# pacargile/ThePayne

Measured on AMD Instinct MI355X. Metric: likelihood-evals/sec (4k-pixel ANN, 512 live points), higher is better.
Workload: dtype f32; 1 GPU; C2: single star per GPU, 4096-pixel 2x300 YST1 ANN, 3600 observed pixels, batch of 512 candidate vectors per step (dynesty live points); batch=512, npix=4096, nobs=3600, stars=1, kernel_variant=0, parallelism=1 star per GPU, no data-path collective, products=2 x fp16 parts, 3 products, fp32 accumulator

## Files before the change

thepayne_amd/csrc/dense_kernels.hpp:

```cpp
#pragma once

#include "sed_core.hpp"
#include "sampler_core.hpp"

typedef float f32x16 __attribute__((ext_vector_type(16)));
typedef float f32x4_t __attribute__((ext_vector_type(4)));

struct DenseParams {
  const float* X; int ldx;
  const float* W; int K;
  const float* Wd; int ldwd;
  int dma_tiles;
  int k_real;
  const float* bias;
  float* Y; int ldy;
  int B, N;
  float bias_shift;
  int act;
  int grid_m, grid_n;
  const double* theta; int ld_theta;
  const float* W0; const float* b0; int n_labels; int act0;
  int K0;
  unsigned short* Yp; const unsigned short* Xp; const unsigned short* Wp;
  int ldp; size_t plane_y, plane_x, plane_w;
  double xmin[PAYNE_MAX_LABELS], xden[PAYNE_MAX_LABELS];
  const unsigned long long* sel; unsigned long long sel_seq;
  const unsigned short* Wp_alt; size_t plane_w_alt; const float* bias_alt; float bias_shift_alt; int N_alt, ldy_alt;
  const float* W_alt;
  int yp_half; float yp_scale;
  const float* rscale; const float* rscale_alt;
  const unsigned short* Wh; size_t plane_wh; const float* rs1; float a0_scale; int h2_tiles;
#ifdef PAYNE_STAMPS
  unsigned long long* stamps;
#endif
};
#define PAYNE_HK_LEAD_PARAMS const void* lead_p0, const float* lead_p1, const float* lead_p2, const float* lead_bias, unsigned lead_i0, unsigned lead_i1, \
                             unsigned lead_i2, int lead_B, unsigned lead_i4, int lead_N
#define PAYNE_HK_LEAD_TYPES const void*, const float*, const float*, const float*, unsigned, unsigned, unsigned, int, unsigned, int
#define PAYNE_D3_LEAD_PARAMS const unsigned long long* lead_sel, const unsigned short* lead_Xp, const unsigned short* lead_Wp, unsigned lead_plane_x, \
                             unsigned lead_plane_w, unsigned lead_grid, int lead_N, int lead_B, int lead_ldp, int lead_K, unsigned lead_sel_seq
#define PAYNE_D3_LEAD_TYPES const unsigned long long*, const unsigned short*, const unsigned short*, unsigned, unsigned, unsigned, int, int, int, int, unsigned
#define PAYNE_D3_LEAD_ARGS(p) (p).sel, (p).Xp, (p).Wp, (unsigned)(p).plane_x, (unsigned)(p).plane_w, ((unsigned)(p).grid_m | ((unsigned)(p).grid_n << 16)), \
                              (p).N, (p).B, (p).ldp, (p).K, (unsigned)(p).sel_seq
#ifdef PAYNE_STAMPS
#ifdef PAYNE_STAMPS_ENDS_ONLY
#define HK_STAMP(k) do { if (((k) == 0 || (k) == 5 || (k) == 15) && p.stamps && threadIdx.x == 0) p.stamps[(size_t)blockIdx.x * 16 + (k)] = __builtin_amdgcn_s_memtime(); } while (0)
#else
#define HK_STAMP(k) do { if (p.stamps && threadIdx.x == 0) p.stamps[(size_t)blockIdx.x * 16 + (k)] = __builtin_amdgcn_s_memtime(); } while (0)
#endif
static unsigned long long* g_hidden_stamps = nullptr;
static unsigned long long* g_dense_stamps = nullptr;
#else
#define HK_STAMP(k) do {} while (0)
#endif

__device__ __forceinline__ float lrelu01(float z) { return fmaxf(z, 0.01f * z); }
__device__ __forceinline__ float sigmoid_f32(float z) {
  const float t = __builtin_amdgcn_fmed3f(-z, -88.0f, 88.0f);
  const float n = __builtin_rintf(t * 1.44269502f);
  float f = __builtin_fmaf(t, 1.44269502f, -n);
  f = __builtin_fmaf(t, 1.92596299e-8f, f);
  const float e = __builtin_amdgcn_ldexpf(__builtin_amdgcn_exp2f(f), (int)n);
  const float d = 1.0f + e;
  float r = __builtin_amdgcn_rcpf(d);
  r = __builtin_fmaf(__builtin_fmaf(-d, r, 1.0f), r, r);
  return z != z ? z : r;
}
__device__ __forceinline__ float act_apply(float z, int act) {
  if (act == PAYNE_ACT_SIGMOID) return sigmoid_f32(z);
  const float l = lrelu01(z);
  return act == PAYNE_ACT_LRELU ? l : z;
}

__device__ __forceinline__ void lds_barrier() { asm volatile("s_waitcnt lgkmcnt(0)\n\ts_barrier" ::: "memory"); }

template <int BM, int BN, int BK>
constexpr size_t dense_lds_bytes() { return (size_t)(2 * (BM + BN) * (BK + 4) + BM * PAYNE_MAX_LABELS) * sizeof(float); }

template <int BM, int BN, int BK, bool FUSE_L0>
__global__ void __launch_bounds__(256) payne_dense_kernel(DenseParams p) {
  constexpr int PITCH = BK + 4;
  constexpr int WM = BM / 2, WN = BN / 2;
  constexpr int TM = WM / 32, TN = WN / 32;
  constexpr int KQ = BK / 4;
  constexpr int A_F4 = BM * KQ / 256, B_F4 = BN * KQ / 256;
  extern __shared__ __attribute__((aligned(16))) float dk_sm[];
  float (*As)[BM * PITCH] = reinterpret_cast<float (*)[BM * PITCH]>(dk_sm);
  float (*Bs)[BN * PITCH] = reinterpret_cast<float (*)[BN * PITCH]>(dk_sm + 2 * BM * PITCH);
  float* Xh = dk_sm + 2 * (BM + BN) * PITCH;

  const int ntiles = p.grid_m * p.grid_n;
  int t = blockIdx.x;
  if ((ntiles & 7) == 0) t = (t & 7) * (ntiles >> 3) + (t >> 3);
  const int m0 = (t % p.grid_m) * BM, n0 = (t / p.grid_m) * BN;
  const int tid = threadIdx.x, lane = tid & 63, wave = tid >> 6;
  const int wm0 = (wave >> 1) * WM, wn0 = (wave & 1) * WN;

  if (FUSE_L0) {
    for (int idx = tid; idx < BM * p.n_labels; idx += 256) {
      const int r = idx / p.n_labels, d = idx - r * p.n_labels, row = m0 + r;
      float v = 0.f;
      if (row < p.B) {
        const double x = p.theta[(size_t)row * p.ld_theta + (d < 4 ? d : 6)];
        v = (float)((x - p.xmin[d]) / p.xden[d] - 0.5);
      }
      Xh[r * PAYNE_MAX_LABELS + d] = v;
// ... 476 lines not shown
#endif
    frags((it + 1) % NS, fn);
    __builtin_amdgcn_sched_barrier(0);
    if (it + AHEAD < nk) issue((it + AHEAD) % NS, (it + AHEAD) * KD);
    __builtin_amdgcn_sched_barrier(0);
  };
  auto epilogue = [&]() {
  if (col < p.N) {
    const bool act_none = __builtin_amdgcn_readfirstlane(p.act == PAYNE_ACT_NONE ? 1 : 0) != 0;
    if (act_none && m0 + 64 <= p.B) {
      const unsigned voff = 4u * ((unsigned)(4 * (lane >> 5)) * (unsigned)p.ldy + (unsigned)col);
      const unsigned char* yb = reinterpret_cast<const unsigned char*>(p.Y + (size_t)(m0 + wm0) * p.ldy);
#pragma unroll
      for (int r = 0; r < 16; ++r) {
        const unsigned char* rowp = yb + (size_t)((r & 3) + 8 * (r >> 2)) * p.ldy * 4;
        d2_store_row(reinterpret_cast<float*>(const_cast<unsigned char*>(rowp + voff)), __builtin_fmaf(acc[r], rs, bv));
      }
    } else if (act_none) {
#pragma unroll
      for (int r = 0; r < 16; ++r) {
        const int row = m0 + wm0 + (r & 3) + 8 * (r >> 2) + 4 * (lane >> 5);
        if (row < p.B) d2_store_row(&p.Y[(size_t)row * p.ldy + col], __builtin_fmaf(acc[r], rs, bv));
      }
    } else {
#pragma unroll
      for (int r = 0; r < 16; ++r) {
        const int row = m0 + wm0 + (r & 3) + 8 * (r >> 2) + 4 * (lane >> 5);
        if (row < p.B) __builtin_nontemporal_store(act_apply(__builtin_fmaf(acc[r], rs, bv), p.act), &p.Y[(size_t)row * p.ldy + col]);
      }
    }
  }
  };
  int it = 0;
#pragma unroll
  for (; it + 2 < nk; it += 2) {
    head(it, f1, f0);
    all_products(f0);
    __builtin_amdgcn_sched_barrier(0);
    head(it + 1, f0, f1);
    all_products(f1);
    __builtin_amdgcn_sched_barrier(0);
  }
  if (it + 1 < nk) {
    head(it, f1, f0);
    all_products(f0);
    last_products(f1);
  } else {
    last_products(f0);
  }
  epilogue();
  HK_STAMP(15);
}

template <int NK> constexpr size_t d2hh_lds_bytes() { return (size_t)NK * 16384 + 3 * 16384; }
template <int NK>
__global__ void __launch_bounds__(512) payne_dense_dma2hh_kernel(PAYNE_D3_LEAD_PARAMS, DenseParams p_) {
  DenseParams p = p_;
  p.sel = lead_sel; p.Xp = lead_Xp; p.Wp = lead_Wp; p.plane_x = lead_plane_x; p.plane_w = lead_plane_w;
  p.grid_m = (int)(lead_grid & 0xffffu); p.grid_n = (int)(lead_grid >> 16); p.N = lead_N; p.B = lead_B; p.ldp = lead_ldp; p.K = lead_K;
  constexpr int KD = 64, ROWB = 2 * KD, CPR = ROWB / 16, RPP = 1024 / ROWB;
  constexpr int PLANE = 64 * ROWB, STAGE = 2 * PLANE;
  constexpr int NSB = 3, AHEAD = 2, KS = KD / 16, NT = 2 * NK;
  constexpr int RING = NK * STAGE;
  auto sw = [](int row) { return (row >> 1) & 7; };
  extern __shared__ __attribute__((aligned(16))) unsigned char d2_sm[];
  if (p.sel != nullptr && (unsigned)*p.sel == lead_sel_seq) {
    p.Wp = p.Wp_alt; p.plane_w = p.plane_w_alt; p.bias = p.bias_alt; p.bias_shift = p.bias_shift_alt; p.N = p.N_alt; p.ldy = p.ldy_alt;
    p.rscale = p.rscale_alt;
  }
  const int ntiles = p.grid_m * p.grid_n;
  int t = blockIdx.x;
  if ((ntiles & 7) == 0) t = (t & 7) * (ntiles >> 3) + (t >> 3);
  const int m0 = (t % p.grid_m) * 64, n0 = (t / p.grid_m) * 128;
  if (n0 >= p.N) return;
  const int tid = threadIdx.x, lane = tid & 63;
  const int wave = __builtin_amdgcn_readfirstlane(tid >> 6);
  const int half = wave >> 2, w4 = wave & 3;
  const int wm0 = (w4 >> 1) * 32, wn0 = 64 * half + (w4 & 1) * 32;
  const int lrow = lane / CPR, lchunk = lane % CPR;
  const unsigned pitch_a = 2u * (unsigned)p.ldp, pitch_b = 2u * (unsigned)p.K;
  const unsigned char* sb1[4]; unsigned vo1[4]; int ds1[4];
  const unsigned char* sb2[4]; unsigned vo2[4]; int ds2[4];
#pragma unroll
  for (int j = 0; j < 4; ++j) {
    {
      const bool isA = j < 2;
      const int pl = j & 1, blk = wave;
      const int row = RPP * blk + lrow, c = lchunk ^ sw(row);
      const int top = isA ? p.B - 1 - m0 : p.N - 1 - n0;
      const int r = (isA ? m0 : n0) + (row < top ? row : top);
      sb1[j] = isA ? reinterpret_cast<const unsigned char*>(p.Xp) + 2 * (size_t)pl * p.plane_x
                   : reinterpret_cast<const unsigned char*>(p.Wp) + 2 * (size_t)pl * p.plane_w;
      vo1[j] = (unsigned)r * (isA ? pitch_a : pitch_b) + 16u * (unsigned)c;
      ds1[j] = pl * PLANE + blk * 1024;
    }
    {
      const int pl = j >> 1, blk = 2 * w4 + (j & 1);
      const int row = RPP * blk + lrow, c = lchunk ^ sw(row);
      const int top = p.N - 1 - n0;
      const int r = n0 + (64 + row < top ? 64 + row : top);
      sb2[j] = reinterpret_cast<const unsigned char*>(p.Wp) + 2 * (size_t)pl * p.plane_w;
      vo2[j] = (unsigned)r * pitch_b + 16u * (unsigned)c;
      ds2[j] = pl * PLANE + blk * 1024;
    }
  }
  auto issue = [&](int q) {
    if (q < NK) {
#pragma unroll
      for (int j = 0; j < 4; ++j)
        __builtin_amdgcn_global_load_lds((const __attribute__((address_space(1))) void*)(sb1[j] + vo1[j] + 2 * KD * q),
                                         (__attribute__((address_space(3))) void*)(d2_sm + (j < 2 ? q * STAGE : RING + (q % NSB) * STAGE) + ds1[j]), 16, 0, 0);
    } else if (half) {
#pragma unroll
      for (int j = 0; j < 4; ++j)
        __builtin_amdgcn_global_load_lds((const __attribute__((address_space(1))) void*)(sb2[j] + vo2[j] + 2 * KD * (q - NK)),
                                         (__attribute__((address_space(3))) void*)(d2_sm + RING + (q % NSB) * STAGE + ds2[j]), 16, 0, 0);
    }
  };
  f32x16 acc;
#pragma unroll
  for (int r = 0; r < 16; ++r) acc[r] = 0.f;
  const int Ra = wm0 + (lane & 31), Rb = (w4 & 1) * 32 + (lane & 31), h = lane >> 5;
  const int sa = sw(Ra), sb = sw(Rb);
  struct Frag { f16x8_t a[KS][2], b[KS][2]; };
  auto frags = [&](int q, Frag& f) {
    const unsigned char* As = d2_sm + (q < NK ? q : q - NK) * STAGE;
    const unsigned char* Bs = d2_sm + RING + (q % NSB) * STAGE;
#pragma unroll
    for (int ks = 0; ks < KS; ++ks) {
      const int c = 2 * ks + h;
#pragma unroll
      for (int pl = 0; pl < 2; ++pl) {
        f.a[ks][pl] = *reinterpret_cast<const f16x8_t*>(As + pl * PLANE + Ra * ROWB + 16 * (c ^ sa));
        f.b[ks][pl] = *reinterpret_cast<const f16x8_t*>(Bs + pl * PLANE + Rb * ROWB + 16 * (c ^ sb));
      }
    }
  };
  auto products = [&](const Frag& f, int ks) {
    acc = __builtin_amdgcn_mfma_f32_32x32x16_f16(f.a[ks][1], f.b[ks][0], acc, 0, 0, 0);
    acc = __builtin_amdgcn_mfma_f32_32x32x16_f16(f.a[ks][0], f.b[ks][1], acc, 0, 0, 0);
    acc = __builtin_amdgcn_mfma_f32_32x32x16_f16(f.a[ks][0], f.b[ks][0], acc, 0, 0, 0);
  };
  const int k_tail = (p.k_real > 0 ? p.k_real : p.K) - (NK - 1) * KD;
  const int ks_last = __builtin_amdgcn_readfirstlane((k_tail + 15) >> 4);
  auto stage_products = [&](const Frag& f, bool last) {
#pragma unroll
    for (int ks = 0; ks < KS; ++ks)
      if (!last || ks < ks_last) products(f, ks);
  };
  const int col = n0 + wn0 + (lane & 31);
  const float bv = p.bias[col < p.N ? col : p.N - 1] - p.bias_shift;
  const float rs = p.rscale[col < p.N ? col : p.N - 1];
  auto epilogue = [&]() {
    if (col >= p.N) return;
    const bool act_none = __builtin_amdgcn_readfirstlane(p.act == PAYNE_ACT_NONE ? 1 : 0) != 0;
    if (act_none && m0 + 64 <= p.B) {
      const unsigned voff = 4u * ((unsigned)(4 * (lane >> 5)) * (unsigned)p.ldy + (unsigned)col);
      const unsigned char* yb = reinterpret_cast<const unsigned char*>(p.Y + (size_t)(m0 + wm0) * p.ldy);
#pragma unroll
      for (int r = 0; r < 16; ++r) {
        const unsigned char* rowp = yb + (size_t)((r & 3) + 8 * (r >> 2)) * p.ldy * 4;
        d2_store_row(reinterpret_cast<float*>(const_cast<unsigned char*>(rowp + voff)), __builtin_fmaf(acc[r], rs, bv));
      }
    } else {
#pragma unroll
      for (int r = 0; r < 16; ++r) {
        const int row = m0 + wm0 + (r & 3) + 8 * (r >> 2) + 4 * (lane >> 5);
        if (row < p.B) {
          const float y = __builtin_fmaf(acc[r], rs, bv);
          __builtin_nontemporal_store(act_none ? y : act_apply(y, p.act), &p.Y[(size_t)row * p.ldy + col]);
        }
      }
    }
  };
  HK_STAMP(0);
  Frag f0, f1;
  if (half == 0) {
    issue(0); issue(1);
    asm volatile("s_waitcnt vmcnt(4)" ::: "memory");
    asm volatile("s_barrier" ::: "memory");
    frags(0, f0);
#pragma unroll
    for (int q = 0; q + 1 < NK; ++q) {
      Frag& fc = (q & 1) ? f1 : f0;
      Frag& fn = (q & 1) ? f0 : f1;
      asm volatile("s_waitcnt vmcnt(0)" ::: "memory");
      asm volatile("s_barrier" ::: "memory");
      HK_STAMP(1 + q);
      frags(q + 1, fn);
      __builtin_amdgcn_sched_barrier(0);
      if (q + AHEAD < NK) issue(q + AHEAD);
      __builtin_amdgcn_sched_barrier(0);
      stage_products(fc, false);
      __builtin_amdgcn_sched_barrier(0);
    }
    asm volatile("s_barrier" ::: "memory");
    stage_products(((NK - 1) & 1) ? f1 : f0, true);
    HK_STAMP(NK);
    epilogue();
    HK_STAMP(15);
    return;
  }
  issue(0); issue(1);
  asm volatile("s_waitcnt vmcnt(4)" ::: "memory");
  asm volatile("s_barrier" ::: "memory");
#pragma unroll
  for (int q = 0; q + 1 < NK; ++q) {
    asm volatile("s_waitcnt vmcnt(0)" ::: "memory");
    asm volatile("s_barrier" ::: "memory");
    issue(q + AHEAD);
  }
  asm volatile("s_waitcnt vmcnt(0)" ::: "memory");
  asm volatile("s_barrier" ::: "memory");
  frags(NK, f0);
  __builtin_amdgcn_sched_barrier(0);
  if (NK + 1 < NT) issue(NK + 1);
  __builtin_amdgcn_sched_barrier(0);
#pragma unroll
  for (int q = NK; q < NT; ++q) {
    Frag& fc = ((q - NK) & 1) ? f1 : f0;
    Frag& fn = ((q - NK) & 1) ? f0 : f1;
    if (q + 1 < NT) {
      asm volatile("s_waitcnt vmcnt(0)" ::: "memory");
      asm volatile("s_barrier" ::: "memory");
      frags(q + 1, fn);
      __builtin_amdgcn_sched_barrier(0);
      if (q + AHEAD < NT) issue(q + AHEAD);
      __builtin_amdgcn_sched_barrier(0);
    }
    stage_products(fc, q == NT - 1);
    __builtin_amdgcn_sched_barrier(0);
  }
  epilogue();
  HK_STAMP(15);
}

constexpr int D3_STAGE = 3 * (64 + 128) * 64;
template <int NS> constexpr size_t d3_lds_bytes() { return (size_t)NS * D3_STAGE; }
template <int NK, int NS, bool PIPE>
__global__ void __launch_bounds__(512) payne_dense_dma3_kernel(PAYNE_D3_LEAD_PARAMS, DenseParams p_) {
  DenseParams p = p_;
  p.sel = lead_sel; p.Xp = lead_Xp; p.Wp = lead_Wp; p.plane_x = lead_plane_x; p.plane_w = lead_plane_w;
  p.grid_m = (int)(lead_grid & 0xffffu); p.grid_n = (int)(lead_grid >> 16); p.N = lead_N; p.B = lead_B; p.ldp = lead_ldp; p.K = lead_K;
  constexpr int D3_NS = NS, AHEAD = PIPE ? D3_NS - 1 : 1;
  static_assert((PIPE && NS >= 3) || (!PIPE && NS == 2 && NK == 0), "ring depth / schedule");
  extern __shared__ __attribute__((aligned(16))) unsigned char d3_sm[];
  if (p.sel != nullptr && (unsigned)*p.sel == lead_sel_seq) {
    p.Wp = p.Wp_alt; p.plane_w = p.plane_w_alt; p.bias = p.bias_alt; p.bias_shift = p.bias_shift_alt; p.N = p.N_alt; p.ldy = p.ldy_alt;
  }
  const int ntiles = p.grid_m * p.grid_n;
  int t = blockIdx.x;
  if ((ntiles & 7) == 0) t = (t & 7) * (ntiles >> 3) + (t >> 3);
  const int m0 = (t % p.grid_m) * 64, n0 = (t / p.grid_m) * 128;
  if (n0 >= p.N) return;
  const int tid = threadIdx.x, lane = tid & 63;
  const int wave = __builtin_amdgcn_readfirstlane(tid >> 6);
  const int wm0 = (wave >> 2) * 32, wn0 = (wave & 3) * 32;
  const bool five = wave < 4;
  const unsigned char* src[5];
  int dst[5];
#pragma unroll
  for (int j = 0; j < 5; ++j) {
    int q = five ? wave * 5 + j : 20 + (wave - 4) * 4 + j;
    if (q > 35) q = 35;
    const bool isA = q < 12;
    const int pl = isA ? q >> 2 : (q - 12) >> 3, blk = isA ? (q & 3) : ((q - 12) & 7);
    const int row = 16 * blk + (lane >> 2);
    const int c = (lane & 3) ^ ((row >> 2) & 3);
    if (isA) {
      const int r = (m0 + row < p.B) ? m0 + row : p.B - 1;
      src[j] = reinterpret_cast<const unsigned char*>(p.Xp + (size_t)pl * p.plane_x + (size_t)r * p.ldp) + 16 * c;
      dst[j] = pl * 4096 + blk * 1024;
    } else {
      const int r = (n0 + row < p.N) ? n0 + row : p.N - 1;
      src[j] = reinterpret_cast<const unsigned char*>(p.Wp + (size_t)pl * p.plane_w + (size_t)r * p.K) + 16 * c;
      dst[j] = 3 * 4096 + pl * 8192 + blk * 1024;
    }
  }
  auto issue = [&](int stage, int k0) {
#pragma unroll
    for (int j = 0; j < 5; ++j)
      if (j < 4 || five)
        __builtin_amdgcn_global_load_lds((const __attribute__((address_space(1))) void*)(src[j] + 2 * k0),
                                         (__attribute__((address_space(3))) void*)(d3_sm + stage * D3_STAGE + dst[j]), 16, 0, 0);
  };
  auto wait_landed = [&](int younger) {
    if (younger <= 0) asm volatile("s_waitcnt vmcnt(0)" ::: "memory");
// ... 1229 lines not shown
```

thepayne_amd/csrc/payne_hip.hip:

```cpp
#include <hip/hip_runtime.h>

#include <chrono>
#include <cstdio>
#include <cstdlib>
#include <cstring>
#include <string>
#include <thread>
#include <vector>

#include "../../include/payne_hip.h"
#include "host_tables.hpp"
#include "post_seq.hpp"
#include "ns_core.hpp"

using namespace payne;

#include "dense_kernels.hpp"

#include "post_kernels.hpp"

#include "sed_kernel.hpp"
#include "select.hpp"

__global__ void payne_photonly_kernel(const double* mags, const double* obs, const double* err, int F, int B, double* lnl) {
  const int b = blockIdx.x * blockDim.x + threadIdx.x;
  if (b < B) lnl[b] = -0.5 * sed_chi2(mags + (size_t)b * F, obs, err, F);
}

static std::string g_create_error;

struct payne_ctx {
  int device = 0;
  payne_opts opts{};
  std::string err;
  std::vector<void*> owned;
  std::vector<void*> obs_owned;
  bool has_model = false;
  int n_layers = 0;
  payne_layer layers[PAYNE_MAX_LAYERS];
  int n_labels = 0;
  double xmin[PAYNE_MAX_LABELS], xden[PAYNE_MAX_LABELS];
  HostTables H;
  PostTables T{};
  float* hid[2] = {nullptr, nullptr};
  int ld_hid = 0;
  float* raw = nullptr;
  const float* w_out_pad = nullptr;
  const float* w_hid_pad[PAYNE_MAX_LAYERS] = {};
  int w_out_kp = 0;
  bool dma_ok = false;
  unsigned short* w_out_p3 = nullptr; unsigned short* hid_p3 = nullptr;
  unsigned short* w_out_p3z = nullptr; const float* bias_z = nullptr; bool freq_ok = false;
  const float* w_out_padz = nullptr;
  unsigned short* w_out_h2 = nullptr; unsigned short* w_out_h2z = nullptr; const float* rscale = nullptr; const float* rscalez = nullptr;
  float act_scale = 0.f;
  unsigned short* w1_h2 = nullptr; const float* rs1 = nullptr; float a0_scale = 0.f; int w1_rows = 0;
  unsigned short* wl_h2[PAYNE_MAX_LAYERS] = {}; const float* rsl[PAYNE_MAX_LAYERS] = {}; float hs[PAYNE_MAX_LAYERS] = {};
  unsigned short* hid_h2[2] = {nullptr, nullptr};
  unsigned long long* chain_flags = nullptr; unsigned long long chain_calls = 0;
  bool freq_rs = false; unsigned long long* rot_flag = nullptr; unsigned long long rot_seq = 0;
  size_t post_lds = 0;
  void (*post_fn_lean)(PAYNE_POST_SIG) = nullptr;
  bool post_tw_lds = false;
  int n_cu = 256;
  bool lean_available = false;
  PostTables* d_T = nullptr;
  post_kernel_fn post_fn = nullptr;
  float* big_ws = nullptr;
  int big_grid = 0;
  bool big_tiled = false;
  bool big_chip = false;
  bool big_chip2 = false;
  bool has_cont = false;
  int cn_layers = 0, cn_npix = 0, cn_ld_hid = 0;
  payne_layer clayers[PAYNE_MAX_LAYERS];
  double cxmin[PAYNE_MAX_LABELS], cxden[PAYNE_MAX_LABELS];
  float* chid[2] = {nullptr, nullptr};
  float* cont_raw = nullptr;
  const double* cont_scale = nullptr;
  const int* cont_idx = nullptr;
  const double* cont_frac = nullptr;
  std::vector<void*> cont_owned;
  bool has_lsf = false;
  const double* d_obs_wave = nullptr;
  const double* lsf = nullptr;
  const double* lsf_wave = nullptr;
  int n_lsf = 0;
  float* lsf_spec = nullptr;
  double* lsf_ws = nullptr;
  float* lsf_fws = nullptr;
  bool lsf_global = false;
  int lsf_chunk = 0;
  std::vector<void*> lsf_owned;
  bool obs_bound = false;
  CandState* prep = nullptr;
  bool has_phot = false, has_obs_phot = false;
  PhotTables P{};
  double* mags_ws = nullptr;
  double *obs_mag = nullptr, *obs_err = nullptr;
  int ncols = 0;
  bool prof = false;
  struct ProfRec { hipEvent_t e0, e1; int kind; };
  std::vector<ProfRec> prof_pool;
// ... 132 lines not shown
  c->T.obs_min = c->H.obs_min;
  c->T.obs_max = c->H.obs_max;
  c->T.ln_obs_min = std::log(c->H.obs_min); c->T.ln_obs_max = std::log(c->H.obs_max);
  c->T.obs_sorted = 1;
  for (int i = 1; i < obs->nobs; ++i) if (!(obs->wave[i] >= obs->wave[i - 1])) { c->T.obs_sorted = 0; break; }
  c->obs_bound = true;
  return sync_tables(c);
}

extern "C" int payne_version(void) { return PAYNE_ABI_VERSION; }

extern "C" const char* payne_last_error(const payne_ctx* ctx) { return ctx ? ctx->err.c_str() : g_create_error.c_str(); }

extern "C" int payne_theta_cols(const payne_ctx* ctx) { return ctx ? ctx->ncols : PAYNE_E_INVALID; }

extern "C" const char* payne_kernel_name(int which) {
  switch (which) {
    case 0: return "payne_dense_kernel";
    case 1: return "payne_post_kernel";
    case 2: return "payne_sed_kernel";
    default: return "";
  }
}

__global__ void payne_activation_kernel(const float* __restrict__ z, int n, int act, float* __restrict__ out) {
  const int i = blockIdx.x * blockDim.x + threadIdx.x;
  if (i < n) out[i] = act_apply(z[i], act);
}
extern "C" int payne_activation_batch(const float* z, int n, int act, float* out, void* stream) {
  if (!z || !out || n < 0 || act < PAYNE_ACT_NONE || act > PAYNE_ACT_SIGMOID) return PAYNE_E_INVALID;
  if (n == 0) return PAYNE_OK;
  hipLaunchKernelGGL(payne_activation_kernel, dim3((n + 255) / 256), dim3(256), 0, reinterpret_cast<hipStream_t>(stream), z, n, act, out);
  return hipGetLastError() == hipSuccess ? PAYNE_OK : PAYNE_E_HIP;
}
extern "C" const char* payne_last_kernel(const payne_ctx* c, int kind) {
  if (c && kind == 4) return c->last_rows_freq ? "frequency" : "pixels";
  return (c && kind >= 0 && kind < 4) ? c->last_kernel[kind] : "";
}

extern "C" void payne_ctx_destroy(payne_ctx* c) {
  if (!c) return;
  int prev = 0;
  (void)hipGetDevice(&prev);
  (void)hipSetDevice(c->device);
  for (void* p : c->owned) (void)hipFree(p);
  for (void* p : c->obs_owned) (void)hipFree(p);
  for (void* p : c->cont_owned) (void)hipFree(p);
  for (void* p : c->lsf_owned) (void)hipFree(p);
  for (auto& r : c->prof_pool) { (void)hipEventDestroy(r.e0); (void)hipEventDestroy(r.e1); }
  (void)hipSetDevice(prev);
  delete c;
}

static hipError_t set_dense_attributes();
static double hidden_amax(const payne_model_desc* m, std::string& why, double* per_layer = nullptr) {
  const int nl = m->n_layers, D = m->n_labels;
  if (nl < 3) { why = "no hidden layer pair"; return 0.0; }
  std::vector<std::vector<float>> W(nl - 1), b(nl - 1);
  for (int l = 0; l + 1 < nl; ++l) {
    const payne_layer& L = m->layers[l];
    W[l].resize((size_t)L.n_out * L.n_in); b[l].resize((size_t)L.n_out);
    if (hipMemcpy(W[l].data(), L.w, W[l].size() * 4, hipMemcpyDeviceToHost) != hipSuccess ||
        hipMemcpy(b[l].data(), L.b, b[l].size() * 4, hipMemcpyDeviceToHost) != hipSuccess) { why = "hipMemcpy"; return 0.0; }
  }
  auto act = [](double z, int a) { return a == PAYNE_ACT_LRELU ? (z > 0 ? z : 0.01 * z) : (a == PAYNE_ACT_SIGMOID ? 1.0 / (1.0 + std::exp(-z)) : z); };
  std::vector<std::vector<double>> pts;
  for (int cidx = 0; cidx < (1 << D); ++cidx) { std::vector<double> x(D); for (int d = 0; d < D; ++d) x[d] = ((cidx >> d) & 1) ? 0.6 : -0.6; pts.push_back(x); }
  pts.push_back(std::vector<double>(D, 0.0));
  unsigned long long st = 0x9E3779B97F4A7C15ull;
  for (int i = 0; i < 64; ++i) {
    std::vector<double> x(D);
    for (int d = 0; d < D; ++d) { st = st * 6364136223846793005ull + 1442695040888963407ull; x[d] = ((double)(st >> 11) / 9007199254740992.0 - 0.5) * 1.2; }
    pts.push_back(x);
  }
  double amax = 0.0;
  std::vector<double> a, y;
  for (const auto& x : pts) {
    a = x;
    for (int l = 0; l + 1 < nl; ++l) {
      const payne_layer& L = m->layers[l];
      y.assign((size_t)L.n_out, 0.0);
      for (int o = 0; o < L.n_out; ++o) {
        double z = b[l][o];
        const float* w = &W[l][(size_t)o * L.n_in];
        for (int k = 0; k < L.n_in; ++k) z += (double)w[k] * a[k];
        y[o] = act(z, L.act);
      }
      a.swap(y);
      if (per_layer) for (double v : a) { if (std::isfinite(v)) per_layer[l] = std::max(per_layer[l], std::fabs(v)); else per_layer[l] = 1e300; }
    }
    for (double v : a) { if (!std::isfinite(v)) { why = "non-finite activation"; return 0.0; } amax = std::max(amax, std::fabs(v)); }
  }
  return amax;
}
static int make_h2_planes(payne_ctx* c, const float* d_w, const std::vector<float>& h_w, int n, int kp, float act_scale,
                          unsigned short** planes, const float** rscale) {
  std::vector<float> sc((size_t)n), rs((size_t)n);
  for (int i = 0; i < n; ++i) {
    float mx = 0.f;
    for (int k = 0; k < kp; ++k) mx = std::max(mx, std::fabs(h_w[(size_t)i * kp + k]));
    int e = 0;
    if (mx > 0.f && std::isfinite(mx)) e = (int)std::floor(std::log2(16384.0 / (double)mx));
    e = std::max(-100, std::min(100, e));
    sc[i] = (float)std::ldexp(1.0, e);
    rs[i] = (float)(std::ldexp(1.0, -e) / (double)act_scale);
  }
  const float* d_sc = nullptr;
// ... 147 lines not shown
  if (!phot->w1 || !phot->b1 || !phot->w2 || !phot->b2 || !phot->w3 || !phot->b3 || !phot->xmin || !phot->xmax)
    return fail(c, PAYNE_E_INVALID, "phot descriptor has NULL members");
  PhotTables& P = c->P;
  const int F = phot->n_filters, H = phot->hidden;
  P.F = F; P.H = H;
  P.w1 = phot->w1; P.b1 = phot->b1; P.b2 = phot->b2; P.w3 = phot->w3; P.b3 = phot->b3;
  for (int d = 0; d < 6; ++d) { P.xmin[d] = phot->xmin[d]; P.xden[d] = phot->xmax[d] - phot->xmin[d]; }
  {
    std::vector<float> w2((size_t)F * H * H), w2t((size_t)F * H * H);
    he = hipMemcpy(w2.data(), phot->w2, w2.size() * 4, hipMemcpyDeviceToHost);
    if (he != hipSuccess) return fail(c, PAYNE_E_HIP, std::string("hipMemcpy(w2): ") + hipGetErrorString(he));
    for (int f = 0; f < F; ++f)
      for (int h = 0; h < H; ++h)
        for (int k = 0; k < H; ++k) w2t[((size_t)f * H + k) * H + h] = w2[((size_t)f * H + h) * H + k];
    if ((rc = upload(c, w2t, &P.w2t, c->owned))) return rc;
  }
  if (phot->hiav) {
    std::vector<double> hv(phot->hiav, phot->hiav + (size_t)F * 5);
    if ((rc = upload(c, hv, &P.hiav, c->owned))) return rc;
  }
  if (phot->obs_mag && phot->obs_err) {
    std::vector<double> m(phot->obs_mag, phot->obs_mag + F), e(phot->obs_err, phot->obs_err + F);
    const double *dm, *de;
    if ((rc = upload(c, m, &dm, c->owned))) return rc;
    if ((rc = upload(c, e, &de, c->owned))) return rc;
    c->obs_mag = const_cast<double*>(dm); c->obs_err = const_cast<double*>(de);
    c->has_obs_phot = true;
  }
  if ((rc = dev_alloc(c, (size_t)opts->b_max * F, &c->mags_ws, c->owned))) return rc;
  if ((size_t)H * 16 > 48 * 1024) {
    he = hipFuncSetAttribute(reinterpret_cast<const void*>(payne_sed_kernel), hipFuncAttributeMaxDynamicSharedMemorySize, H * 16);
    if (he != hipSuccess) return fail(c, PAYNE_E_HIP, std::string("hipFuncSetAttribute(sed): ") + hipGetErrorString(he));
  }
  c->has_phot = true;
  return PAYNE_OK;
}

extern "C" int payne_ctx_create(const payne_model_desc* model, const payne_obs_desc* obs, const payne_phot_desc* phot,
                                const payne_opts* opts, int device, payne_ctx** out) {
  if (!out) return fail(nullptr, PAYNE_E_INVALID, "out is NULL");
  *out = nullptr;
  if (!opts || opts->b_max <= 0) return fail(nullptr, PAYNE_E_INVALID, "opts.b_max must be > 0");
  if (opts->npoly < 0 || opts->npoly > PAYNE_MAX_POLY) return fail(nullptr, PAYNE_E_INVALID, "opts.npoly out of range");
  if (!model && !phot) return fail(nullptr, PAYNE_E_INVALID, "need a spectral model and/or a photometric model");
  hipError_t he = hipSetDevice(device);
  if (he != hipSuccess) return fail(nullptr, PAYNE_E_HIP, std::string("hipSetDevice: ") + hipGetErrorString(he));
  payne_ctx* c = new payne_ctx();
  c->device = device;
  { int ncu = 0; if (hipDeviceGetAttribute(&ncu, hipDeviceAttributeMultiprocessorCount, device) == hipSuccess && ncu > 0) c->n_cu = ncu; }
  c->opts = *opts;
  c->ncols = 8 + opts->npoly + 4;
  int rc = PAYNE_OK;
  auto bail = [&](int code) { g_create_error = c->err; payne_ctx_destroy(c); return code; };
  he = set_dense_attributes();
  if (he != hipSuccess) return bail(fail(c, PAYNE_E_HIP, std::string("hipFuncSetAttribute(dense): ") + hipGetErrorString(he)));

  if (model) {
    if (model->n_layers < 2 || model->n_layers > PAYNE_MAX_LAYERS) return bail(fail(c, PAYNE_E_INVALID, "model.n_layers must be 2..8"));
    if (model->n_labels < 1 || model->n_labels > PAYNE_MAX_LABELS) return bail(fail(c, PAYNE_E_INVALID, "model.n_labels must be 1..5"));
    if (!model->xmin || !model->xmax || !model->wavelength) return bail(fail(c, PAYNE_E_INVALID, "model.xmin/xmax/wavelength missing"));
    if (model->layers[0].n_in != model->n_labels) return bail(fail(c, PAYNE_E_INVALID, "first layer n_in != n_labels"));
    if (model->layers[model->n_layers - 1].n_out != model->npix) return bail(fail(c, PAYNE_E_INVALID, "last layer n_out != npix"));
    int maxh = 0;
    if ((rc = adopt_layers(c, model, c->layers, c->owned, "", &maxh))) return bail(rc);
    if ((rc = create_dense_operands(c, model, opts, maxh))) return bail(rc);
    c->n_layers = model->n_layers;
    c->n_labels = model->n_labels;
    for (int d = 0; d < model->n_labels; ++d) { c->xmin[d] = model->xmin[d]; c->xden[d] = model->xmax[d] - model->xmin[d]; }
    rc = build_model_tables(model->wavelength, model->npix, c->H);
    if (rc == -1) return bail(fail(c, PAYNE_E_INVALID, "model.npix must be >= 16"));
    if (rc == -2) return bail(fail(c, PAYNE_E_INVALID, "model.wavelength must be strictly increasing"));
    if (c->H.n1 > (1 << 20)) return bail(fail(c, PAYNE_E_UNSUPPORTED, "npix > 2^20"));
    PostTables& T = c->T;
    fill_model_scalars(c->H, T);
    T.r_ann = model->resolution; T.npoly = opts->npoly;
    if ((rc = upload(c, c->H.vs_tab32, &T.vs_tab, c->owned))) return bail(rc);
    T.vs_tab += 1;
    if ((rc = dev_alloc(c, 1, &c->d_T, c->owned))) return bail(rc);
    if ((rc = upload(c, c->H.lnlam, &T.lnlam, c->owned))) return bail(rc);
    if ((rc = upload(c, c->H.lam, &T.lam, c->owned))) return bail(rc);
    if ((rc = upload(c, c->H.tw, &T.tw, c->owned))) return bail(rc);
    if ((rc = upload(c, c->H.twf, &T.twf, c->owned))) return bail(rc);
    if ((rc = upload(c, c->H.rs1_idx, &T.rs1_idx, c->owned))) return bail(rc);
    if ((rc = upload(c, c->H.rs1_frac, &T.rs1_frac, c->owned))) return bail(rc);
    if ((rc = upload(c, c->H.bk1_idx, &T.bk1_idx, c->owned))) return bail(rc);
    if ((rc = upload(c, c->H.bk1_frac, &T.bk1_frac, c->owned))) return bail(rc);
    c->ld_hid = (maxh + 31) & ~31;
    if (model->n_layers > 2) {
      if ((rc = dev_alloc(c, (size_t)opts->b_max * c->ld_hid, &c->hid[0], c->owned))) return bail(rc);
      if ((rc = dev_alloc(c, (size_t)opts->b_max * c->ld_hid, &c->hid[1], c->owned))) return bail(rc);
      if (c->w_out_p3 && (rc = dev_alloc(c, (size_t)3 * opts->b_max * c->ld_hid, &c->hid_p3, c->owned))) return bail(rc);
    }
    if ((rc = dev_alloc(c, (size_t)opts->b_max * std::max(model->npix, T.n1 <= 16384 ? T.n1 : 0), &c->raw, c->owned, false))) return bail(rc);
    if ((rc = dev_alloc(c, (size_t)opts->b_max, &c->prep, c->owned, false))) return bail(rc);
    if (T.n1 > 16384) {
      c->big_grid = opts->b_max < 256 ? opts->b_max : 256;
      c->big_chip2 = T.n1 == kChip2N1 && c->H.geo && !(opts->variant & PAYNE_V_BIG_WORKSPACE);
      if ((rc = dev_alloc(c, (size_t)c->big_grid * (c->big_chip2 ? 4 : 2) * T.n1, &c->big_ws, c->owned, false))) return bail(rc);
      if (c->big_chip2) {
        he = hipFuncSetAttribute(reinterpret_cast<const void*>(payne_post_chip2_kernel), hipFuncAttributeMaxDynamicSharedMemorySize,
                                 (int)kChipLdsBytes);
        if (he != hipSuccess) return bail(fail(c, PAYNE_E_HIP, std::string("hipFuncSetAttribute(chip2): ") + hipGetErrorString(he)));
      }
      c->big_tiled = true;
      c->big_chip = T.n1 == kChipN1 && c->H.geo && !(opts->variant & PAYNE_V_BIG_WORKSPACE);
      if (c->big_chip) {
        he = hipFuncSetAttribute(reinterpret_cast<const void*>(payne_post_chip_kernel), hipFuncAttributeMaxDynamicSharedMemorySize,
// ... 78 lines not shown
  }
  if ((rc = upload(c, scale, &c->cont_scale, c->cont_owned))) return rc;
  if ((rc = upload(c, idx, &c->cont_idx, c->cont_owned))) return rc;
  if ((rc = upload(c, frac, &c->cont_frac, c->cont_owned))) return rc;
  c->has_cont = true;
  return PAYNE_OK;
}

static int set_lsf_impl(payne_ctx* c, const double* lsf_wave, const double* lsf, int n) {
  if (!c) return PAYNE_E_INVALID;
  if (!c->has_model) return fail(c, PAYNE_E_INVALID, "context has no spectral model");
  DeviceScope ds(c);
  for (void* p : c->lsf_owned) (void)hipFree(p);
  c->lsf_owned.clear();
  c->has_lsf = false;
  if (!lsf) return PAYNE_OK;
  if (!c->obs_bound) return fail(c, PAYNE_E_INVALID, "bind the observed grid before its LSF vector");
  if (!lsf_wave && n != c->T.nobs) return fail(c, PAYNE_E_INVALID, "the LSF vector must have one entry per observed pixel");
  if (lsf_wave && n < 2) return fail(c, PAYNE_E_INVALID, "an LSF vector on its own wavelengths needs at least two entries");
  for (int i = 0; i < n; ++i)
    if (!(lsf[i] > 0.0)) return fail(c, PAYNE_E_INVALID, "LSF dispersions must be positive");
  if (lsf_wave)
    for (int i = 1; i < n; ++i)
      if (!(lsf_wave[i] > lsf_wave[i - 1])) return fail(c, PAYNE_E_INVALID, "the LSF vector's wavelengths must be strictly increasing");
  std::vector<double> v(lsf, lsf + n);
  int rc;
  if ((rc = upload(c, v, &c->lsf, c->lsf_owned))) return rc;
  c->n_lsf = n;
  c->lsf_wave = c->d_obs_wave;
  if (lsf_wave) {
    std::vector<double> w(lsf_wave, lsf_wave + n);
    if ((rc = upload(c, w, &c->lsf_wave, c->lsf_owned))) return rc;
  }
  c->lsf_global = c->T.n1 > 8192 || (c->opts.variant & PAYNE_V_LSF_GLOBAL);
  c->lsf_chunk = c->lsf_global ? std::min(c->opts.b_max, 256) : c->opts.b_max;
  if ((rc = dev_alloc(c, (size_t)c->lsf_chunk * c->T.npix, &c->lsf_spec, c->lsf_owned, false))) return rc;
  if ((rc = dev_alloc(c, (size_t)c->lsf_chunk * (2 * (size_t)c->T.npix + c->T.n1), &c->lsf_ws, c->lsf_owned, false))) return rc;
  if (c->lsf_global) {
    if ((rc = dev_alloc(c, (size_t)c->lsf_chunk * 2 * fft_buf_floats(c->T.n1), &c->lsf_fws, c->lsf_owned, false))) return rc;
  } else {
    const size_t lds = (size_t)c->T.n1 * 8 + 2 * (size_t)fft_buf_floats(c->T.n1) * 4 + (256 + 8) * 8;
    hipError_t he = hipFuncSetAttribute(reinterpret_cast<const void*>(payne_lsf_kernel<false>), hipFuncAttributeMaxDynamicSharedMemorySize, (int)lds);
    if (he != hipSuccess) return fail(c, PAYNE_E_HIP, std::string("hipFuncSetAttribute: ") + hipGetErrorString(he));
  }
  c->has_lsf = true;
  return PAYNE_OK;
}
extern "C" int payne_ctx_set_lsf(payne_ctx* c, const double* lsf, int n) { return set_lsf_impl(c, nullptr, lsf, n); }
extern "C" int payne_ctx_set_lsf_on(payne_ctx* c, const double* lsf_wave, const double* lsf, int n) {
  if (c && lsf && !lsf_wave) return fail(c, PAYNE_E_INVALID, "lsf_wave is NULL");
  return set_lsf_impl(c, lsf_wave, lsf, n);
}

static hipError_t set_dense_attributes() {
  hipError_t e = hipSuccess;
  auto set = [&](const void* f, size_t lds) {
    const hipError_t r = hipFuncSetAttribute(f, hipFuncAttributeMaxDynamicSharedMemorySize, (int)lds);
    if (e == hipSuccess) e = r;
  };
#define PAYNE_SET_T(K, ARGS, ...) set(reinterpret_cast<const void*>(PAYNE_UNPAREN K), __VA_ARGS__);
#define PAYNE_SET_F(K, ...) set(reinterpret_cast<const void*>(K), __VA_ARGS__);
  PAYNE_DENSE_KERNELS(PAYNE_SET_T, PAYNE_SET_F)
  return e;
}

template <int BM, int BN, int BK, bool FUSE>
static void launch_dense(DenseParams& p, hipStream_t s) {
  p.grid_m = (p.B + BM - 1) / BM;
  p.grid_n = (p.N + BN - 1) / BN;
#ifdef PAYNE_STAMPS
  p.stamps = FUSE ? nullptr : g_dense_stamps;
#endif
  PAYNE_LAUNCH_DENSE((payne_dense_kernel<BM, BN, BK, FUSE>), dim3(p.grid_m * p.grid_n), dim3(256), s, p);
}

template <int BK, int NK, int NS, bool PIPE>
static void launch_out_dma_nk(DenseParams& p, hipStream_t s) {
  constexpr int WN = 4;
  PAYNE_LAUNCH_DENSE((payne_dense_dma_kernel<WN, BK, NK, NS, PIPE>), dim3(p.grid_m * p.grid_n), dim3(128 * WN), s, p);
}
struct OutPlan {
  OutForm form = OutForm::Generic;
  int grid_m = 0, grid_n = 0;
  bool sel = false;
  bool big = false;
  bool own_cu = false;
  bool fixed = false;
  bool bk64 = false;
  bool halves = false;
  bool split_w = false;
};
static void launch_out_dma(payne_ctx* c, DenseParams& p, hipStream_t s, const OutPlan& plan) {
  p.k_real = p.K;
  p.W = c->w_out_pad; p.K = c->w_out_kp;
  p.grid_m = plan.grid_m; p.grid_n = plan.grid_n;
#ifdef PAYNE_STAMPS
  p.stamps = g_dense_stamps;
#endif
  if (plan.bk64) {
    if (plan.fixed) launch_out_dma_nk<64, 5, 3, true>(p, s); else launch_out_dma_nk<64, 0, 3, true>(p, s);
  } else if (plan.own_cu) {
    if (plan.fixed) launch_out_dma_nk<32, 10, 4, true>(p, s); else launch_out_dma_nk<32, 0, 4, true>(p, s);
  } else {
    launch_out_dma_nk<32, 0, 3, false>(p, s);
  }
}

static void launch_out_planes(payne_ctx* c, DenseParams& p, hipStream_t s, const OutPlan& plan, bool freq) {
  const bool h2 = plan.form == OutForm::H2;
  p.k_real = p.K;
// ... 69 lines not shown
    else PAYNE_LAUNCH_DENSE((payne_dense_hidden_kernel<true, PAYNE_MAX_LABELS>), grid, block, s, PAYNE_HK_ARGS);
  }
#undef PAYNE_HK_ARGS
}

struct NetRef {
  const payne_layer* layers; int n_layers; int n_labels; const double* xmin; const double* xden;
  float* const* hid; int ld_hid; float* out; int ld_out; float out_shift;
  bool spectral;
  bool freq = false;
  bool sel = false;
};
static NetRef spectral_net(const payne_ctx* c) {
  return NetRef{c->layers, c->n_layers, c->n_labels, c->xmin, c->xden, c->hid, c->ld_hid, c->raw, c->T.npix, kBase, true};
}
static NetRef continuum_net(const payne_ctx* c) {
  return NetRef{c->clayers, c->cn_layers, c->n_labels, c->cxmin, c->cxden, c->chid, c->cn_ld_hid, c->cont_raw, c->cn_npix, 0.f, false};
}
struct BatchRows {
  const float* rows = nullptr; int ld = 0;
  bool freq = false;
  bool sel = false; unsigned long long rot_seq = 0;
  const CandState* prep = nullptr;
  bool spec = false;
};
struct SpecReq { const WalkTail* walk; const WalkState* w; int step, K; };
static OutForm out_form(const payne_ctx* c, const NetRef& N) {
  OutForm f = wanted_out_form(c->opts.variant);
  if (!(N.spectral && c->dma_ok && c->ld_hid >= c->w_out_kp)) return OutForm::Generic;
  if (f >= OutForm::Bf16x3 && !(c->w_out_p3 && c->hid_p3)) f = OutForm::F32Dma;
  if (f == OutForm::H2) {
    const unsigned long long plane_w = 2ull * (unsigned long long)std::max(N.layers[N.n_layers - 1].n_out, c->T.n1) * (unsigned long long)c->w_out_kp;
    const unsigned long long plane_x = 2ull * (unsigned long long)c->opts.b_max * (unsigned long long)c->ld_hid;
    if (plane_w >= (1ull << 31) || plane_x >= (1ull << 31) || !c->w_out_h2 || !(c->act_scale > 0.f)) f = OutForm::Bf16x3;
  }
  return f;
}
static OutPlan plan_out(const payne_ctx* c, const NetRef& N, int B) {
  const unsigned v = c->opts.variant;
  const int kp = c->w_out_kp, n_out = N.layers[N.n_layers - 1].n_out;
  OutPlan o; o.sel = N.sel;
  const int n_launch = o.sel ? c->T.n1 : n_out;
  o.form = out_form(c, N);
  if (o.form == OutForm::H2 && N.freq && !c->w_out_h2z) o.form = OutForm::Bf16x3;
  if (o.form == OutForm::Generic) return o;
  o.grid_m = (B + 63) / 64; o.grid_n = (n_launch + 127) / 128;
  o.own_cu = o.grid_m * o.grid_n <= c->n_cu;
  o.fixed = kp == 320 && !(v & PAYNE_V_OUT_ROLLED);
  if (o.form == OutForm::F32Dma) { o.bk64 = kp % 64 == 0 && (v & PAYNE_V_OUT_BK64); return o; }
  if (B % B3_TM == 0 && n_launch % B3_TN == 0 && (B / B3_TM) * (n_launch / B3_TN) >= 2 * c->n_cu && !(v & PAYNE_V_OUT_SMALL_TILES) && !o.sel) {
    o.big = true; o.grid_m = B / B3_TM; o.grid_n = n_launch / B3_TN;
    return o;
  }
  if (o.form == OutForm::H2) o.halves = o.fixed && o.own_cu && !(v & PAYNE_V_OUT_WHOLE_TILE);
  else o.split_w = o.fixed && o.own_cu && (N.freq ? c->w_out_padz : c->w_out_pad) && !(v & PAYNE_V_OUT_PLANES) && (!o.sel || c->w_out_pad);
  return o;
}
static int run_net(payne_ctx* c, const NetRef& N, const OutPlan& plan, const double* theta, int B, double instr_factor, hipStream_t s,
                   BatchRows* R = nullptr, bool* sed = nullptr, const SpecReq& spec = SpecReq{}) {
  const int n = N.n_layers;
  const bool use3 = plan.form >= OutForm::Bf16x3, use2h = plan.form == OutForm::H2;
  for (int l = 1; l < n; ++l) {
    DenseParams p{};
    const payne_layer& L = N.layers[l];
    const bool last = (l == n - 1);
    p.W = L.w; p.K = L.n_in; p.bias = L.b; p.N = L.n_out; p.B = B; p.act = L.act;
    p.bias_shift = last ? N.out_shift : 0.f;
    p.Y = last ? N.out : N.hid[(l - 1) & 1];
    p.ldy = last ? N.ld_out : N.ld_hid;
    if (use3 && l == n - 2) {
      p.Yp = c->hid_p3; p.plane_y = (size_t)c->opts.b_max * c->ld_hid; p.ldp = c->ld_hid;
      if (use2h) { p.yp_half = 1; p.yp_scale = c->act_scale; }
    }
    const bool chain = N.spectral && c->hid_h2[0] && c->w1_h2 && c->w1_rows == N.layers[1].n_out;
    if (chain && !last && l + 1 <= n - 2 && c->wl_h2[l + 1]) {
      p.Yp = c->hid_h2[(l - 1) & 1]; p.plane_y = (size_t)c->opts.b_max * 304; p.ldp = 304; p.yp_half = 1; p.yp_scale = c->hs[l];
    }
    ProfScope ps(c, s, last ? 0 : 3);
    if (l == 1) {
      const payne_layer& L0 = N.layers[0];
      p.theta = theta; p.ld_theta = c->ncols;
      p.W0 = L0.w; p.b0 = L0.b; p.n_labels = N.n_labels; p.act0 = L0.act; p.K0 = L0.n_out;
      for (int d = 0; d < N.n_labels; ++d) { p.xmin[d] = N.xmin[d]; p.xden[d] = N.xden[d]; }
      PrepArgs pa{};
      pa.T = c->T; pa.T.raw_freq = N.freq ? 1 : 0; pa.instr_factor = instr_factor;
      pa.out = (N.spectral && c->prep && c->obs_bound && !(c->opts.variant & PAYNE_V_NO_PREP)) ? c->prep : nullptr;
      if (plan.sel) { pa.rot_flag = c->rot_flag; pa.rot_seq = R->rot_seq; }
      if (!last && sed && *sed && N.spectral && sed_tile_ok(c->P.H) && !(c->opts.variant & PAYNE_V_SED_OWN_LAUNCH)) {
        pa.P = c->P; pa.sed_mags = c->mags_ws; pa.sed_off = 8 + c->opts.npoly; pa.sed_photscale = c->opts.photscale;
        *sed = false;
      }
      const int spec_K = (!last && N.spectral && spec.walk && pa.out && c->lean_available && !c->big_ws) ? spec.K : 0;
      if (spec_K) { pa.spec_walk = spec.walk; pa.spec_w = *spec.w; pa.spec_step = spec.step; }
      if (!last && N.spectral && c->w_hid_pad[1] && N.ld_hid >= HK_PITCH) { p.Wd = c->w_hid_pad[1]; p.ldwd = N.ld_hid; }
      if (!last && N.spectral && p.Wd && c->w1_h2 && c->w1_rows == p.N && p.K <= 304 &&
          (unsigned long long)B * (unsigned)c->ncols * 8ull < (1ull << 31)) {
        p.h2_tiles = 1; p.Wh = c->w1_h2; p.plane_wh = (size_t)c->w1_rows * 304; p.rs1 = c->rs1; p.a0_scale = c->a0_scale;
      }
      if (!last && !hk_lead_fits(p.B, p.N, p.K, p.K0, 0, p.ldwd, p.ld_theta, spec_K))
        return fail(c, PAYNE_E_UNSUPPORTED, "batch x hidden width beyond what the hidden-layer kernel's packed arguments hold (65 535 tiles of 32 x 32)");
      if (last) launch_dense<64, 64, 32, true>(p, s);
      else launch_hidden<true>(p, pa, s, c->n_cu, spec_K, (c->opts.variant & PAYNE_V_HID_WAVES4) != 0);
      if (!last && R) { R->prep = pa.out; R->spec = spec_K != 0; }
    } else if (!last && chain && use3 && l == 2 && n - 2 >= 3 && c->chain_flags && (c->opts.variant & PAYNE_V_HID_CHAIN) &&
               ((c->opts.b_max + 31) / 32) * ((N.layers[2].n_out + 31) / 32) <= 2 * c->n_cu && n - 3 <= kChainMax &&
               [&] { for (int q = 2; q <= n - 2; ++q) if (!c->wl_h2[q]) return false; return true; }()) {
      ChainParams cp{};
// ... 1311 lines not shown
```

Baseline: 18.91 million likelihood-evals/s.

## Deepen dma2hh prefetch with full W staging area and partial vmcnt waits

```diff
diff --git a/thepayne_amd/csrc/dense_kernels.hpp b/thepayne_amd/csrc/dense_kernels.hpp
--- a/thepayne_amd/csrc/dense_kernels.hpp
+++ b/thepayne_amd/csrc/dense_kernels.hpp
@@ -44,14 +44,16 @@
                               (p).N, (p).B, (p).ldp, (p).K, (unsigned)(p).sel_seq
 #ifdef PAYNE_STAMPS
 #ifdef PAYNE_STAMPS_ENDS_ONLY
-#define HK_STAMP(k) do { if (((k) == 0 || (k) == 5 || (k) == 15) && p.stamps && threadIdx.x == 0) p.stamps[(size_t)blockIdx.x * 16 + (k)] = __builtin_amdgcn_s_memtime(); } while (0)
+#define HK_STAMP_AT(k, t) do { if (((k) == 0 || (k) == 5 || (k) == 15) && p.stamps && threadIdx.x == (t)) p.stamps[(size_t)blockIdx.x * 16 + (k)] = __builtin_amdgcn_s_memtime(); } while (0)
 #else
-#define HK_STAMP(k) do { if (p.stamps && threadIdx.x == 0) p.stamps[(size_t)blockIdx.x * 16 + (k)] = __builtin_amdgcn_s_memtime(); } while (0)
+#define HK_STAMP_AT(k, t) do { if (p.stamps && threadIdx.x == (t)) p.stamps[(size_t)blockIdx.x * 16 + (k)] = __builtin_amdgcn_s_memtime(); } while (0)
 #endif
+#define HK_STAMP(k) HK_STAMP_AT(k, 0)
 static unsigned long long* g_hidden_stamps = nullptr;
 static unsigned long long* g_dense_stamps = nullptr;
 #else
 #define HK_STAMP(k) do {} while (0)
+#define HK_STAMP_AT(k, t) do {} while (0)
 #endif
 
 __device__ __forceinline__ float lrelu01(float z) { return fmaxf(z, 0.01f * z); }
@@ -634,7 +636,28 @@
   HK_STAMP(15);
 }
 
-template <int NK> constexpr size_t d2hh_lds_bytes() { return (size_t)NK * 16384 + 3 * 16384; }
+#ifndef D2HH_AHEAD
+#define D2HH_AHEAD 5
+#endif
+template <int NK> constexpr size_t d2hh_lds_bytes() { return (size_t)NK * 16384 + (size_t)NK * 16384; }
+template <int NK> constexpr int d2hh_issued(int s) {
+  constexpr int NT = 2 * NK, AHEAD = D2HH_AHEAD;
+  int last = (AHEAD < NK ? AHEAD : NK) - 1;
+  for (int b = 0; b <= s; ++b) {
+    int upto = b + AHEAD < NK + b - 1 ? b + AHEAD : NK + b - 1;
+    if (b >= NK || upto > NT - 1) upto = NT - 1;
+    if (upto > last) last = upto;
+  }
+  return last;
+}
+__device__ __forceinline__ void d2hh_wait_vm(int n) {
+  if (n <= 0) asm volatile("s_waitcnt vmcnt(0)" ::: "memory");
+  else if (n == 4) asm volatile("s_waitcnt vmcnt(4)" ::: "memory");
+  else if (n == 8) asm volatile("s_waitcnt vmcnt(8)" ::: "memory");
+  else if (n == 12) asm volatile("s_waitcnt vmcnt(12)" ::: "memory");
+  else if (n == 16) asm volatile("s_waitcnt vmcnt(16)" ::: "memory");
+  else asm volatile("s_waitcnt vmcnt(0)" ::: "memory");
+}
 template <int NK>
 __global__ void __launch_bounds__(512) payne_dense_dma2hh_kernel(PAYNE_D3_LEAD_PARAMS, DenseParams p_) {
   DenseParams p = p_;
@@ -642,8 +665,8 @@
   p.grid_m = (int)(lead_grid & 0xffffu); p.grid_n = (int)(lead_grid >> 16); p.N = lead_N; p.B = lead_B; p.ldp = lead_ldp; p.K = lead_K;
   constexpr int KD = 64, ROWB = 2 * KD, CPR = ROWB / 16, RPP = 1024 / ROWB;
   constexpr int PLANE = 64 * ROWB, STAGE = 2 * PLANE;
-  constexpr int NSB = 3, AHEAD = 2, KS = KD / 16, NT = 2 * NK;
-  constexpr int RING = NK * STAGE;
+  constexpr int KS = KD / 16, NT = 2 * NK;
+  constexpr int WAREA = NK * STAGE;
   auto sw = [](int row) { return (row >> 1) & 7; };
   extern __shared__ __attribute__((aligned(16))) unsigned char d2_sm[];
   if (p.sel != nullptr && (unsigned)*p.sel == lead_sel_seq) {
@@ -691,13 +714,18 @@
 #pragma unroll
       for (int j = 0; j < 4; ++j)
         __builtin_amdgcn_global_load_lds((const __attribute__((address_space(1))) void*)(sb1[j] + vo1[j] + 2 * KD * q),
-                                         (__attribute__((address_space(3))) void*)(d2_sm + (j < 2 ? q * STAGE : RING + (q % NSB) * STAGE) + ds1[j]), 16, 0, 0);
+                                         (__attribute__((address_space(3))) void*)(d2_sm + (j < 2 ? 0 : WAREA) + q * STAGE + ds1[j]), 16, 0, 0);
     } else if (half) {
 #pragma unroll
       for (int j = 0; j < 4; ++j)
         __builtin_amdgcn_global_load_lds((const __attribute__((address_space(1))) void*)(sb2[j] + vo2[j] + 2 * KD * (q - NK)),
-                                         (__attribute__((address_space(3))) void*)(d2_sm + RING + (q % NSB) * STAGE + ds2[j]), 16, 0, 0);
-    }
+                                         (__attribute__((address_space(3))) void*)(d2_sm + WAREA + (q - NK) * STAGE + ds2[j]), 16, 0, 0);
+    }
+  };
+  auto issue_upto = [&](int from, int upto) {
+#pragma unroll
+    for (int q = 0; q < NT; ++q)
+      if (q > from && q <= upto) issue(q);
   };
   f32x16 acc;
 #pragma unroll
@@ -707,7 +735,7 @@
   struct Frag { f16x8_t a[KS][2], b[KS][2]; };
   auto frags = [&](int q, Frag& f) {
     const unsigned char* As = d2_sm + (q < NK ? q : q - NK) * STAGE;
-    const unsigned char* Bs = d2_sm + RING + (q % NSB) * STAGE;
+    const unsigned char* Bs = As + WAREA;
 #pragma unroll
     for (int ks = 0; ks < KS; ++ks) {
       const int c = 2 * ks + h;
@@ -731,9 +759,12 @@
       if (!last || ks < ks_last) products(f, ks);
   };
   const int col = n0 + wn0 + (lane & 31);
-  const float bv = p.bias[col < p.N ? col : p.N - 1] - p.bias_shift;
-  const float rs = p.rscale[col < p.N ? col : p.N - 1];
+  const float b_req = p.bias[col < p.N ? col : p.N - 1];
+  const float rs_req = p.rscale[col < p.N ? col : p.N - 1];
   auto epilogue = [&]() {
+    float b_in = b_req, rs = rs_req;
+    asm volatile("" : "+v"(b_in), "+v"(rs));
+    const float bv = b_in - p.bias_shift;
     if (col >= p.N) return;
     const bool act_none = __builtin_amdgcn_readfirstlane(p.act == PAYNE_ACT_NONE ? 1 : 0) != 0;
     if (act_none && m0 + 64 <= p.B) {
@@ -757,64 +788,73 @@
   };
   HK_STAMP(0);
   Frag f0, f1;
+  issue_upto(-1, d2hh_issued<NK>(-1));
   if (half == 0) {
-    issue(0); issue(1);
-    asm volatile("s_waitcnt vmcnt(4)" ::: "memory");
+    constexpr int P1 = NK - 1;
+    d2hh_wait_vm(4 * ((d2hh_issued<NK>(-1) < P1 ? d2hh_issued<NK>(-1) : P1) - 0));
     asm volatile("s_barrier" ::: "memory");
     frags(0, f0);
+    __builtin_amdgcn_sched_barrier(0);
+    issue_upto(d2hh_issued<NK>(-1), d2hh_issued<NK>(0) < P1 ? d2hh_issued<NK>(0) : P1);
+    __builtin_amdgcn_sched_barrier(0);
 #pragma unroll
     for (int q = 0; q + 1 < NK; ++q) {
       Frag& fc = (q & 1) ? f1 : f0;
       Frag& fn = (q & 1) ? f0 : f1;
-      asm volatile("s_waitcnt vmcnt(0)" ::: "memory");
+      const int had = d2hh_issued<NK>(q) < P1 ? d2hh_issued<NK>(q) : P1, get = d2hh_issued<NK>(q + 1) < P1 ? d2hh_issued<NK>(q + 1) : P1;
+      d2hh_wait_vm(4 * (had - (q + 1)));
+      asm volatile("s_waitcnt lgkmcnt(0)" ::: "memory");
       asm volatile("s_barrier" ::: "memory");
       HK_STAMP(1 + q);
       frags(q + 1, fn);
       __builtin_amdgcn_sched_barrier(0);
-      if (q + AHEAD < NK) issue(q + AHEAD);
+      issue_upto(had, get);
       __builtin_amdgcn_sched_barrier(0);
       stage_products(fc, false);
       __builtin_amdgcn_sched_barrier(0);
     }
+    asm volatile("s_waitcnt lgkmcnt(0)" ::: "memory");
     asm volatile("s_barrier" ::: "memory");
     stage_products(((NK - 1) & 1) ? f1 : f0, true);
     HK_STAMP(NK);
     epilogue();
-    HK_STAMP(15);
     return;
   }
-  issue(0); issue(1);
-  asm volatile("s_waitcnt vmcnt(4)" ::: "memory");
+  d2hh_wait_vm(4 * (d2hh_issued<NK>(-1) - 0));
   asm volatile("s_barrier" ::: "memory");
+  issue_upto(d2hh_issued<NK>(-1), d2hh_issued<NK>(0));
 #pragma unroll
   for (int q = 0; q + 1 < NK; ++q) {
-    asm volatile("s_waitcnt vmcnt(0)" ::: "memory");
+    d2hh_wait_vm(4 * (d2hh_issued<NK>(q) - (q + 1)));
     asm volatile("s_barrier" ::: "memory");
-    issue(q + AHEAD);
-  }
-  asm volatile("s_waitcnt vmcnt(0)" ::: "memory");
+    issue_upto(d2hh_issued<NK>(q), d2hh_issued<NK>(q + 1));
+  }
   asm volatile("s_barrier" ::: "memory");
-  frags(NK, f0);
-  __builtin_amdgcn_sched_barrier(0);
-  if (NK + 1 < NT) issue(NK + 1);
-  __builtin_amdgcn_sched_barrier(0);
+  issue_upto(d2hh_issued<NK>(NK - 1), NT - 1);
 #pragma unroll
   for (int q = NK; q < NT; ++q) {
     Frag& fc = ((q - NK) & 1) ? f1 : f0;
     Frag& fn = ((q - NK) & 1) ? f0 : f1;
+    if (q == NK) {
+      d2hh_wait_vm(4 * (NT - 1 - (NK + 1 < NT - 1 ? NK + 1 : NT - 1)));
+      asm volatile("s_barrier" ::: "memory");
+      HK_STAMP_AT(NK + 1, 256);
+      frags(NK, f0);
+    }
     if (q + 1 < NT) {
-      asm volatile("s_waitcnt vmcnt(0)" ::: "memory");
-      asm volatile("s_barrier" ::: "memory");
+      if (((q + 1 - NK) & 1) == 0) {
+        d2hh_wait_vm(4 * (NT - 1 - (q + 2 < NT - 1 ? q + 2 : NT - 1)));
+        asm volatile("s_barrier" ::: "memory");
+        HK_STAMP_AT(NK + 1 + (q + 1 - NK) / 2, 256);
+      }
       frags(q + 1, fn);
       __builtin_amdgcn_sched_barrier(0);
-      if (q + AHEAD < NT) issue(q + AHEAD);
-      __builtin_amdgcn_sched_barrier(0);
     }
     stage_products(fc, q == NT - 1);
     __builtin_amdgcn_sched_barrier(0);
   }
   epilogue();
-  HK_STAMP(15);
+  HK_STAMP_AT(15, 256);
 }
 
 constexpr int D3_STAGE = 3 * (64 + 128) * 64;
diff --git a/thepayne_amd/csrc/payne_hip.hip b/thepayne_amd/csrc/payne_hip.hip
--- a/thepayne_amd/csrc/payne_hip.hip
+++ b/thepayne_amd/csrc/payne_hip.hip
@@ -49,6 +49,7 @@
   const float* w_hid_pad[PAYNE_MAX_LAYERS] = {};
   int w_out_kp = 0;
   bool dma_ok = false;
+  bool out_halves_ok = false;
   unsigned short* w_out_p3 = nullptr; unsigned short* hid_p3 = nullptr;
   unsigned short* w_out_p3z = nullptr; const float* bias_z = nullptr; bool freq_ok = false;
   const float* w_out_padz = nullptr;
@@ -287,7 +288,7 @@
   delete c;
 }
 
-static hipError_t set_dense_attributes();
+static hipError_t set_dense_attributes(bool* halves_ok);
 static double hidden_amax(const payne_model_desc* m, std::string& why, double* per_layer = nullptr) {
   const int nl = m->n_layers, D = m->n_labels;
   if (nl < 3) { why = "no hidden layer pair"; return 0.0; }
@@ -541,7 +542,7 @@
   c->ncols = 8 + opts->npoly + 4;
   int rc = PAYNE_OK;
   auto bail = [&](int code) { g_create_error = c->err; payne_ctx_destroy(c); return code; };
-  he = set_dense_attributes();
+  he = set_dense_attributes(&c->out_halves_ok);
   if (he != hipSuccess) return bail(fail(c, PAYNE_E_HIP, std::string("hipFuncSetAttribute(dense): ") + hipGetErrorString(he)));
 
   if (model) {
@@ -726,10 +727,13 @@
   return set_lsf_impl(c, lsf_wave, lsf, n);
 }
 
-static hipError_t set_dense_attributes() {
+static hipError_t set_dense_attributes(bool* halves_ok) {
   hipError_t e = hipSuccess;
+  *halves_ok = true;
+  const void* halves = reinterpret_cast<const void*>(payne_dense_dma2hh_kernel<5>);
   auto set = [&](const void* f, size_t lds) {
     const hipError_t r = hipFuncSetAttribute(f, hipFuncAttributeMaxDynamicSharedMemorySize, (int)lds);
+    if (f == halves && r != hipSuccess) { *halves_ok = false; (void)hipGetLastError(); return; }
     if (e == hipSuccess) e = r;
   };
 #define PAYNE_SET_T(K, ARGS, ...) set(reinterpret_cast<const void*>(PAYNE_UNPAREN K), __VA_ARGS__);
@@ -905,7 +909,7 @@
     o.big = true; o.grid_m = B / B3_TM; o.grid_n = n_launch / B3_TN;
     return o;
   }
-  if (o.form == OutForm::H2) o.halves = o.fixed && o.own_cu && !(v & PAYNE_V_OUT_WHOLE_TILE);
+  if (o.form == OutForm::H2) o.halves = o.fixed && o.own_cu && c->out_halves_ok && !(v & PAYNE_V_OUT_WHOLE_TILE);
   else o.split_w = o.fixed && o.own_cu && (N.freq ? c->w_out_padz : c->w_out_pad) && !(v & PAYNE_V_OUT_PLANES) && (!o.sel || c->w_out_pad);
   return o;
 }
```

Measured after the change: 18.54 million likelihood-evals/s. -2.0%, worse.
